# KaHIP/KaMinPar

Hardware: NVIDIA H100
Metric: lp_edges_per_second (higher is better)
Workload: dtype int32

## Files before the change

kaminpar_b200/csrc/lp_sweep.cuh:

```cuda
#pragma once

#include "lp_device.cuh"
#include "lp_sortnet.cuh"

namespace kmp {

template <int MODE>
__device__ __forceinline__ void emit_proposal(const SweepArgs &a, uint32_t idx, uint32_t u, uint32_t target,
                                              int32_t uw) {
  a.mv_u[idx] = u;
  a.mv_t[idx] = target;
  if (!a.accumulate) {
    return;
  }
  if (MODE == 0) {
    atomicAdd(&a.incoming[target], uw);
  } else {
    const uint32_t lvl = ladder_level(bijective32(u, a.base_commit));
    atomicAdd(&a.hist[target * kLadderLevels + lvl], uw);
  }
}

__device__ __forceinline__ void block_count_flush(const SweepArgs &a, unsigned long long edges,
                                                  unsigned long long nodes) {
  for (int o = 16; o > 0; o >>= 1) {
    edges += __shfl_xor_sync(kFull, edges, o);
    nodes += __shfl_xor_sync(kFull, nodes, o);
  }
  if ((threadIdx.x & 31) == 0 && nodes != 0) {
    atomicAdd(&a.counters[0], edges);
    atomicAdd(&a.counters[kCounterNodesOffset], nodes);
  }
}

template <bool P64>
__device__ __forceinline__ typename LabG<P64>::word load_labg(const SweepArgs &a, uint32_t v) {
  return static_cast<const typename LabG<P64>::word *>(a.labg)[v];
}

template <int R> struct ThreadRow {
  uint32_t u, beg, deg;
  uint32_t v[R > 0 ? R : 1];
};
template <int R> __device__ __forceinline__ void load_row(const SweepArgs &a, ThreadRow<R> &r) {
  r.beg = a.xadj[r.u];
  const uint32_t deg = a.xadj[r.u + 1] - r.beg;
  r.deg = deg > a.max_num_neighbors ? a.max_num_neighbors : deg;
#pragma unroll
  for (int j = 0; j < R; ++j) {
    r.v[j] = j < static_cast<int>(r.deg) ? a.adjncy[r.beg + j] : 0u;
  }
}

template <int MODE, bool EW, bool P64, int N, int R>
__device__ __forceinline__ bool sweep_thread_vertex(const SweepArgs &a, const ThreadRow<R> &r, bool flag,
                                                    unsigned long long &edges, unsigned long long &nodes,
                                                    uint32_t &target, int32_t &uw) {
  const uint32_t u = r.u;
  const uint32_t own = a.label[u];
  uw = a.vwgt != nullptr ? a.vwgt[u] : 1;
  const int32_t own_w = a.weight[own];
  uint32_t keys[N];
  int32_t ws[N];
  bool hit = false;
#pragma unroll
  for (int j = 0; j < N; ++j) {
    keys[j] = kEmpty;
    ws[j] = 0;
    if (j < static_cast<int>(r.deg)) {
      const uint32_t v = R > 0 ? r.v[j] : a.adjncy[r.beg + j];
      const typename LabG<P64>::word g = load_labg<P64>(a, v);
      hit = hit || stamp_hit(LabG<P64>::stamp(g), a.window);
      bool ok = true;
      if (MODE == 1 && a.communities != nullptr) {
        ok = a.communities[u] == a.communities[v];
      }
      if (ok) {
        keys[j] = LabG<P64>::label(g);
        ws[j] = EW ? a.adjwgt[r.beg + j] : 1;
      }
    }
  }
  if (!(flag || hit)) {
    return false;
  }
  edges += r.deg;
  nodes += 1;
  if (a.active != nullptr && flag) {
    a.active[u] = 0;
  }
  bool skip = false;
  if (MODE == 1) {
    const int32_t mn = a.min_w != nullptr ? a.min_w[own] : 0;
    skip = (own_w - uw) < mn;
  }
  const bool store_fav = (MODE == 0) && (uw == own_w) && (own_w <= a.max_cluster_weight / 2);
  Cand best = cand_none(), fav = cand_none();
  if (!skip) {
    sort_registers<N, EW>(keys, ws);
    bool lazy_done = false;
    if (MODE == 0) {
      Cand top = cand_none();
      int32_t run = 0;
#pragma unroll
      for (int j = 0; j < N; ++j) {
        run += EW ? ws[j] : 1;
        const bool last = (j == N - 1) || (keys[j + 1 < N ? j + 1 : j] != keys[j]);
        if (last) {
          const int32_t rating = run;
          run = 0;
          if (keys[j] != kEmpty && rating > 0) {
            if (rating >= top.gain) {
              const Cand x{rating, 0, tie_hash(a.base_tie, u, keys[j]), keys[j]};
              if (cand_better<0>(x, top)) {
                top = x;
              }
            }
            if (store_fav && rating >= fav.gain) {
              const Cand y{rating, 0, tie_hash(a.base_fav, u, keys[j]), keys[j]};
              if (cand_better<0>(y, fav)) {
                fav = y;
              }
            }
          }
        }
      }
      bool top_ok = true;
      if (top.gain > 0) {
        top_ok = (a.weight[top.key] + uw <= a.max_cluster_weight) || (top.key == own);
        if (a.communities != nullptr) {
          top_ok = top_ok && (a.communities[top.key] == a.communities[own]);
        }
      }
      if (top_ok) {
        best = top;
        lazy_done = true;
      }
    }
    if (!lazy_done) {
      int32_t run = 0;
#pragma unroll
      for (int j = 0; j < N; ++j) {
        run += EW ? ws[j] : 1;
        const bool last = (j == N - 1) || (keys[j + 1 < N ? j + 1 : j] != keys[j]);
        if (last) {
          const int32_t rating = run;
          run = 0;
          if (keys[j] != kEmpty) {
            Cand f;
            const Cand c = eval_candidate<MODE>(a, u, own, uw, own_w, keys[j], rating, MODE == 0 ? false : store_fav, f);
            if (cand_better<MODE>(c, best)) {
              best = c;
            }
          }
        }
      }
    }
  }
  return finish_vertex<MODE>(a, u, own, store_fav, best, fav, target);
}

template <int MODE>
__device__ __forceinline__ void emit_cta_iteration(const SweepArgs &a, bool proposes, uint32_t u, uint32_t target,
                                                   int32_t uw, uint32_t it, uint32_t (&s_cnt)[2][8],
                                                   uint32_t (&s_base)[2]) {
  const unsigned ballot = __ballot_sync(kFull, proposes);
  const int lane = threadIdx.x & 31;
  const int wib = threadIdx.x >> 5;
  const int par = it & 1;
  if (lane == 0) {
    s_cnt[par][wib] = static_cast<uint32_t>(__popc(ballot));
  }
  __syncthreads();
  if (threadIdx.x == 0) {
    uint32_t total = 0;
    for (int w = 0; w < 8; ++w) {
      total += s_cnt[par][w];
    }
    s_base[par] = total != 0 ? atomicAdd(a.mover_count, total) : 0u;
  }
  __syncthreads();
  if (proposes) {
    uint32_t idx = s_base[par] + __popc(ballot & ((1u << lane) - 1u));
    for (int w = 0; w < wib; ++w) {
      idx += s_cnt[par][w];
    }
    emit_proposal<MODE>(a, idx, u, target, uw);
  }
}

template <int MODE, bool EW, bool P64, int N> __global__ void __launch_bounds__(256) sweep_thread(const SweepArgs a) {
  __shared__ uint32_t s_cnt[2][8];
  __shared__ uint32_t s_base[2];
  unsigned long long edges = 0, nodes = 0;
  const uint32_t stride = gridDim.x * blockDim.x;
  const uint32_t bound = (a.list_size + 255u) & ~255u;
  uint32_t it = 0;
  for (uint32_t i = blockIdx.x * blockDim.x + threadIdx.x; i < bound; i += stride, ++it) {
    bool proposes = false;
    uint32_t target = 0;
    int32_t uw = 1;
    ThreadRow<0> r;
    r.u = 0;
    if (i < a.list_size) {
      r.u = a.list[i];
      const bool flag = a.active == nullptr || a.active[r.u] != 0;
      if (flag || a.pull) {
        load_row<0>(a, r);
        proposes = sweep_thread_vertex<MODE, EW, P64, N>(a, r, flag, edges, nodes, target, uw);
      }
    }
    emit_cta_iteration<MODE>(a, proposes, r.u, target, uw, it, s_cnt, s_base);
  }
  block_count_flush(a, edges, nodes);
}

__device__ __forceinline__ uint32_t pow2_ceil(uint32_t x) {
  return x <= 1 ? 1u : (1u << (32 - __clz(static_cast<int>(x - 1))));
}

__device__ __forceinline__ void table_add(uint32_t *keys, int32_t *vals, uint32_t mask, bool direct, uint32_t key,
                                          int32_t w) {
  uint32_t slot = direct ? key : (lowbias32(key) & mask);
  while (true) {
    const uint32_t prev = atomicCAS(&keys[slot], kEmpty, key);
    if (prev == kEmpty || prev == key) {
      atomicAdd(&vals[slot], w);
      return;
    }
    slot = (slot + 1) & mask;
  }
}

template <int T> struct TeamSync {
  static __device__ __forceinline__ void sync(int id) {
    if (T == 32) {
      __syncwarp();
    } else {
      asm volatile("bar.sync %0, %1;" ::"r"(id), "r"(T) : "memory");
    }
  }
  static __device__ __forceinline__ bool any(int id, bool p) {
    if (T == 32) {
      __syncwarp();
      return __any_sync(kFull, p);
    } else {
      int r;
      asm volatile(
          "{\n"
          ".reg .pred q, r;\n"
          "setp.ne.s32 q, %3, 0;\n"
          "bar.red.or.pred r, %1, %2, q;\n"
          "selp.s32 %0, 1, 0, r;\n"
          "}\n"
          : "=r"(r)
          : "r"(id), "r"(T), "r"(static_cast<int>(p))
          : "memory");
      return r != 0;
    }
  }
};

template <int MODE, int T>
__device__ __forceinline__ Cand team_argmax(int id, int tid, Cand c, Cand *s_red) {
  Cand r = warp_argmax<MODE>(kFull, c);
  if (T == 32) {
    return r;
  }
  TeamSync<T>::sync(id);
  if ((tid & 31) == 0) {
    s_red[tid >> 5] = r;
  }
  TeamSync<T>::sync(id);
  Cand x = cand_none();
  if ((tid & 31) < T / 32) {
    x = s_red[tid & 31];
  }
  return warp_argmax<MODE>(kFull, x);
}

template <bool V16> struct TeamVals;
template <> struct TeamVals<false> {
  using word = int32_t;
  static constexpr int kBytesPerSlot = 4;
  static __device__ __forceinline__ void add(word *v, uint32_t slot, int32_t w) { atomicAdd(&v[slot], w); }
  static __device__ __forceinline__ int32_t get(const word *v, uint32_t slot) { return v[slot]; }
  static __device__ __forceinline__ void clear(word *v, uint32_t slot) { v[slot] = 0; }
};
template <> struct TeamVals<true> {
  using word = uint32_t;
  static constexpr int kBytesPerSlot = 2;
  static __device__ __forceinline__ void add(word *v, uint32_t slot, int32_t w) {
    atomicAdd(&v[slot >> 1], static_cast<uint32_t>(w) << ((slot & 1u) * 16u));
  }
  static __device__ __forceinline__ int32_t get(const word *v, uint32_t slot) {
    return static_cast<int32_t>((v[slot >> 1] >> ((slot & 1u) * 16u)) & 0xFFFFu);
  }
  static __device__ __forceinline__ void clear(word *v, uint32_t slot) { reinterpret_cast<uint16_t *>(v)[slot] = 0; }
};

template <bool V16, bool EW>
__device__ __forceinline__ bool team_table_add(uint32_t *keys, typename TeamVals<V16>::word *vals, uint32_t mask,
                                               bool direct, uint32_t key, int32_t w, uint32_t &slot) {
  slot = direct ? key : (lowbias32(key) & mask);
  while (true) {
    const uint32_t prev = atomicCAS(&keys[slot], kEmpty, key);
    if (!EW && prev == kEmpty) {
      return true;
    }
    if (prev == kEmpty || prev == key) {
      TeamVals<V16>::add(vals, slot, w);
      return prev == kEmpty;
    }
    slot = (slot + 1) & mask;
  }
}
template <bool V16, bool EW>
__device__ __forceinline__ int32_t team_rating(const typename TeamVals<V16>::word *vals, uint32_t slot) {
  return TeamVals<V16>::get(vals, slot) + (EW ? 0 : 1);
}

template <int T> constexpr int team_ctas_per_sm() { return T == 32 ? 6 : T == 1024 ? 1 : 3; }

template <int MODE, bool EW, bool P64, int T, int SLOTS, int TEAMS, bool V16 = false>
__global__ void __launch_bounds__(T *TEAMS, team_ctas_per_sm<T>()) sweep_team(const SweepArgs a) {
  static_assert((SLOTS & (SLOTS - 1)) == 0, "table size must be a power of two");
  static_assert(SLOTS <= 65536, "claim lists hold 16-bit slot indices");
  static_assert(!(V16 && EW), "16-bit ratings need unit edge weights");
  using TV = TeamVals<V16>;
  constexpr int kListCap = SLOTS / 2;
  extern __shared__ __align__(16) unsigned char smem_raw[];
  __shared__ Cand s_red_all[TEAMS][T > 32 ? T / 32 : 1];
  __shared__ uint16_t s_list_all[TEAMS][kListCap];
  __shared__ uint32_t s_next[TEAMS], s_claims[TEAMS];
  __shared__ unsigned long long s_edges[TEAMS], s_nodes[TEAMS];
  const int team = threadIdx.x / T;
  const int tid = threadIdx.x % T;
  const int lane = threadIdx.x & 31;
  const int bar = 1 + team;
  uint32_t *keys = reinterpret_cast<uint32_t *>(smem_raw) + static_cast<size_t>(team) * SLOTS;
  typename TV::word *vals = reinterpret_cast<typename TV::word *>(
      smem_raw + sizeof(uint32_t) * SLOTS * TEAMS + static_cast<size_t>(team) * SLOTS * TV::kBytesPerSlot);
  Cand *s_red = s_red_all[team];
  uint16_t *list = s_list_all[team];
  for (int s = tid; s < SLOTS; s += T) {
    keys[s] = kEmpty;
    TV::clear(vals, s);
  }
  uint32_t next = 0;
  unsigned long long edges = 0, nodes = 0;
  if (tid == 0) {
    next = atomicAdd(a.queue, 1u);
    if (T > 32) {
      s_edges[team] = 0;
      s_nodes[team] = 0;
    }
  }
  TeamSync<T>::sync(bar);
  while (true) {
    uint32_t i;
    if (T == 32) {
      i = __shfl_sync(kFull, next, 0);
    } else {
      if (tid == 0) {
        s_next[team] = next;
        s_claims[team] = 0;
      }
      TeamSync<T>::sync(bar);
      i = s_next[team];
    }
    if (i >= a.list_size) {
      break;
    }
    if (tid == 0) {
      next = atomicAdd(a.queue, 1u);
    }
    const uint32_t u = a.list[i];
    const bool flag = a.active == nullptr || a.active[u] != 0;
    if (!flag && !a.pull) {
      TeamSync<T>::sync(bar);
      continue;
    }
    const uint32_t beg = a.xadj[u];
    uint32_t deg = a.xadj[u + 1] - beg;
    if (deg > a.max_num_neighbors) {
      deg = a.max_num_neighbors;
    }
    const uint32_t own = a.label[u];
    const int32_t uw = a.vwgt != nullptr ? a.vwgt[u] : 1;
    const int32_t own_w = a.weight[own];
    bool skip = false;
    if (MODE == 1) {
      const int32_t mn = a.min_w != nullptr ? a.min_w[own] : 0;
      skip = (own_w - uw) < mn;
    }
    const bool direct = a.num_labels <= static_cast<uint32_t>(SLOTS);
    bool hit = false;
    uint32_t claims = 0;
    constexpr int B = 4;
    for (uint32_t e0 = 0; e0 < deg; e0 += T * B) {
      uint32_t kb[B];
      int32_t wb[B];
      uint32_t vb[B];
#pragma unroll
      for (int j = 0; j < B; ++j) {
        const uint32_t e = e0 + j * T + tid;
        vb[j] = e < deg ? a.adjncy[beg + e] : kEmpty;
        wb[j] = (EW && e < deg) ? a.adjwgt[beg + e] : 1;
      }
#pragma unroll
      for (int j = 0; j < B; ++j) {
        kb[j] = kEmpty;
        if (vb[j] != kEmpty) {
          const typename LabG<P64>::word g = load_labg<P64>(a, vb[j]);
          hit = hit || stamp_hit(LabG<P64>::stamp(g), a.window);
          bool ok = !skip;
          if (MODE == 1 && a.communities != nullptr) {
            ok = ok && a.communities[u] == a.communities[vb[j]];
          }
          if (ok) {
            kb[j] = LabG<P64>::label(g);
          }
        }
      }
      uint32_t sl[B];
      unsigned claimed[B];
#pragma unroll
      for (int j = 0; j < B; ++j) {
        sl[j] = 0;
        claimed[j] = __ballot_sync(kFull, kb[j] != kEmpty && team_table_add<V16, EW>(keys, vals, SLOTS - 1, direct,
                                                                                     kb[j], wb[j], sl[j]));
      }
      uint32_t n = 0;
#pragma unroll
      for (int j = 0; j < B; ++j) {
        n += __popc(claimed[j]);
      }
      if (n != 0) {
        uint32_t base = claims;
        if (T == 32) {
          claims += n;
        } else {
          if (lane == 0) {
            base = atomicAdd(&s_claims[team], n);
          }
          base = __shfl_sync(kFull, base, 0);
        }
        const unsigned below = (1u << lane) - 1u;
#pragma unroll
        for (int j = 0; j < B; ++j) {
          if ((claimed[j] >> lane) & 1u) {
            list[base + __popc(claimed[j] & below)] = static_cast<uint16_t>(sl[j]);
          }
          base += __popc(claimed[j]);
        }
      }
    }
    const bool any_hit = TeamSync<T>::any(bar, hit);
    const bool act = flag || any_hit;
    const uint32_t nc = T == 32 ? claims : s_claims[team];
    const bool store_fav = (MODE == 0) && (uw == own_w) && (own_w <= a.max_cluster_weight / 2);
    Cand best = cand_none(), fav = cand_none();
    if (act) {
      Cand c = cand_none(), f = cand_none();
      if (MODE == 0) {
        for (uint32_t l = tid; l < nc; l += T) {
          const uint32_t s = list[l];
          const uint32_t k = keys[s];
          const int32_t r = team_rating<V16, EW>(vals, s);
          if (r >= c.gain) {
            Cand x{r, 0, tie_hash(a.base_tie, u, k), k};
            if (cand_better<0>(x, c)) {
              c = x;
            }
          }
          if (store_fav && r >= f.gain) {
            Cand y{r, 0, tie_hash(a.base_fav, u, k), k};
            if (cand_better<0>(y, f)) {
              f = y;
            }
          }
        }
        const Cand top = team_argmax<0, T>(bar, tid, c, s_red);
        if (store_fav) {
          fav = team_argmax<0, T>(bar, tid, f, s_red);
        }
        bool top_ok = true;
        if (top.gain > 0) {
          top_ok = (a.weight[top.key] + uw <= a.max_cluster_weight) || (top.key == own);
          if (a.communities != nullptr) {
            top_ok = top_ok && (a.communities[top.key] == a.communities[own]);
          }
        }
        if (top_ok) {
          best = top;
        } else {
          Cand cb = cand_none();
          for (uint32_t l0 = 0; l0 < nc; l0 += T * 4) {
            uint32_t kk[4];
            int32_t rr[4], ww[4];
#pragma unroll
            for (int j = 0; j < 4; ++j) {
              const uint32_t l = l0 + j * T + tid;
              const uint32_t s = l < nc ? list[l] : 0u;
              kk[j] = l < nc ? keys[s] : kEmpty;
              rr[j] = l < nc ? team_rating<V16, EW>(vals, s) : 0;
            }
#pragma unroll
            for (int j = 0; j < 4; ++j) {
              ww[j] = kk[j] != kEmpty ? a.weight[kk[j]] : 0;
            }
#pragma unroll
            for (int j = 0; j < 4; ++j) {
              if (kk[j] != kEmpty) {
                Cand ff;
                const Cand cc = eval_candidate_w<0>(a, u, own, uw, own_w, kk[j], rr[j], ww[j], false, ff);
                if (cand_better<0>(cc, cb)) {
                  cb = cc;
                }
              }
            }
          }
          best = team_argmax<0, T>(bar, tid, cb, s_red);
        }
      } else {
        for (uint32_t l = tid; l < nc; l += T) {
          const uint32_t s = list[l];
          const uint32_t k = keys[s];
          Cand ff;
          const Cand cc = eval_candidate_w<1>(a, u, own, uw, own_w, k, team_rating<V16, EW>(vals, s), a.weight[k], false, ff);
          if (cand_better<1>(cc, c)) {
            c = cc;
          }
        }
        best = team_argmax<1, T>(bar, tid, c, s_red);
      }
    }
    for (uint32_t l = tid; l < nc; l += T) {
      const uint32_t s = list[l];
      keys[s] = kEmpty;
      TV::clear(vals, s);
    }
    if (act && tid == 0) {
      if (T == 32) {
        edges += deg;
        nodes += 1;
      } else {
        s_edges[team] += deg;
        s_nodes[team] += 1;
      }
      if (a.active != nullptr && flag) {
        a.active[u] = 0;
      }
      uint32_t target;
      if (finish_vertex<MODE>(a, u, own, store_fav, best, fav, target)) {
        const uint32_t idx = atomicAdd(a.mover_count, 1u);
        emit_proposal<MODE>(a, idx, u, target, uw);
      }
    }
    TeamSync<T>::sync(bar);
  }
  if (T > 32 && tid == 0) {
    edges = s_edges[team];
    nodes = s_nodes[team];
  }
  if (tid == 0 && nodes != 0) {
    atomicAdd(&a.counters[0], edges);
    atomicAdd(&a.counters[kCounterNodesOffset], nodes);
  }
}

constexpr int kChunkEdges = 2048;
constexpr int kSliceEdges = 256;
constexpr int kSliceTableSlots = 512;
constexpr int kChunkThreads = 256;
constexpr uint32_t kBucketCap = 512;
constexpr uint32_t kBucketTargetFill = 256;
constexpr uint32_t kSelTableSlots = 1024;
constexpr int kSelWarps = 4;

struct HubOverflow {
  uint32_t bucket;
  uint32_t key;
  int32_t rating;
  uint32_t pad;
};

struct HubArgs {
  const uint32_t *__restrict__ item_entry;
  const uint32_t *__restrict__ item_chunk;
  const uint32_t *__restrict__ item_u;
  const uint32_t *__restrict__ item_beg;
  const uint32_t *__restrict__ item_deg;
  uint32_t num_items;
  const uint32_t *__restrict__ table_off;
  unsigned long long *__restrict__ g_tab;
  uint32_t *__restrict__ cursor;
  HubOverflow *__restrict__ ovf;
  uint32_t *__restrict__ ovf_count;
  uint32_t ovf_cap;
  uint32_t bucket_cap;
  uint32_t sel_limit;
  uint32_t stage_adjncy;
  const uint32_t *__restrict__ sel_entry;
  const uint32_t *__restrict__ sel_piece;
  uint32_t num_sel_items;
  const uint32_t *__restrict__ sel_begin;
  Cand *__restrict__ part_best;
  Cand *__restrict__ part_fav;
  uint32_t rank, world;
  uint32_t *__restrict__ queue;
  uint32_t *__restrict__ hit;
  uint32_t *__restrict__ lab;
  const uint32_t *__restrict__ lab_off;
  const uint32_t *__restrict__ item_cls;
};

__host__ __device__ __forceinline__ uint32_t hub_buckets(uint32_t full_degree) {
  const uint32_t need = (full_degree + kBucketTargetFill - 1) / kBucketTargetFill;
  uint32_t p = 1;
  while (p < need) {
    p <<= 1;
  }
  return p;
}

__device__ __forceinline__ uint32_t smem_u32(const void *p) {
  return static_cast<uint32_t>(__cvta_generic_to_shared(p));
}
__device__ __forceinline__ void mbar_init(uint64_t *bar, uint32_t count) {
  asm volatile("mbarrier.init.shared::cta.b64 [%0], %1;" ::"r"(smem_u32(bar)), "r"(count) : "memory");
}
__device__ __forceinline__ void mbar_arrive_expect_tx(uint64_t *bar, uint32_t bytes) {
  asm volatile("mbarrier.arrive.expect_tx.shared::cta.b64 _, [%0], %1;" ::"r"(smem_u32(bar)), "r"(bytes) : "memory");
}
__device__ __forceinline__ void mbar_wait(uint64_t *bar, uint32_t parity) {
  asm volatile(
      "{\n"
      ".reg .pred p;\n"
      "WAIT_LOOP:\n"
      "mbarrier.try_wait.parity.shared::cta.b64 p, [%0], %1;\n"
      "@p bra DONE;\n"
      "bra WAIT_LOOP;\n"
      "DONE:\n"
      "}\n" ::"r"(smem_u32(bar)),
      "r"(parity)
      : "memory");
}
__device__ __forceinline__ void tma_load_1d(void *dst_smem, const void *src_gmem, uint32_t bytes, uint64_t *bar) {
  asm volatile("cp.async.bulk.shared::cluster.global.mbarrier::complete_tx::bytes [%0], [%1], %2, [%3];" ::"r"(
                   smem_u32(dst_smem)),
               "l"(src_gmem), "r"(bytes), "r"(smem_u32(bar))
               : "memory");
}

struct HubItem {
  uint32_t valid;
  uint32_t u;
  uint32_t entry;
  uint32_t full_deg;
  uint32_t gbeg, gend;
  uint32_t a0;
  uint32_t staged;
};

__device__ __forceinline__ void mbar_arrive(uint64_t *bar) {
  asm volatile("mbarrier.arrive.shared::cta.b64 _, [%0];" ::"r"(smem_u32(bar)) : "memory");
}

constexpr int kHubStages = 2;
constexpr int kHubConsumerWarps = kChunkThreads / 32;
constexpr int kHubThreads = kChunkThreads + 32;
constexpr int kHubScatterSmem = kHubConsumerWarps * kSliceTableSlots * 8;

template <int MODE, bool EW, bool P64>
__global__ void __launch_bounds__(kHubThreads, 4) sweep_hub_scatter(const SweepArgs a, const HubArgs hb, uint32_t m_total) {
  extern __shared__ __align__(16) unsigned char smem_raw[];
  constexpr int kAllSlots = kHubConsumerWarps * kSliceTableSlots;
  uint32_t *all_keys = reinterpret_cast<uint32_t *>(smem_raw);
  int32_t *all_vals = reinterpret_cast<int32_t *>(smem_raw + sizeof(uint32_t) * kAllSlots);
  __shared__ __align__(16) uint32_t s_adj[kHubStages][kChunkEdges + 8];
  __shared__ __align__(8) uint64_t s_full[kHubStages];
  __shared__ __align__(8) uint64_t s_empty[kHubStages];
  __shared__ HubItem s_item[kHubStages];
  const int lane = threadIdx.x & 31;
  const int wib = threadIdx.x >> 5;
  if (threadIdx.x == 0) {
    for (int s = 0; s < kHubStages; ++s) {
      mbar_init(&s_full[s], 1);
      mbar_init(&s_empty[s], kHubConsumerWarps);
    }
    asm volatile("fence.mbarrier_init.release.cluster;" ::: "memory");
  }
  for (int s = threadIdx.x; s < kAllSlots; s += kHubThreads) {
    all_keys[s] = kEmpty;
    all_vals[s] = 0;
  }
  __syncthreads();

  if (wib == kHubConsumerWarps) {
    if (lane == 0) {
      for (uint32_t k = 0;; ++k) {
        const int stage = static_cast<int>(k % kHubStages);
        const uint32_t round = k / kHubStages;
        mbar_wait(&s_empty[stage], (round & 1u) ^ 1u);
        const uint32_t it = atomicAdd(hb.queue, 1u);
        HubItem d{};
        d.valid = 0;
        if (it >= hb.num_items) {
          d.valid = 2;
          s_item[stage] = d;
          mbar_arrive(&s_full[stage]);
          break;
        }
        const uint32_t entry = hb.item_entry[it];
        const uint32_t u = hb.item_u[it];
        const uint32_t beg0 = hb.item_beg[it];
        const uint32_t full_deg = hb.item_deg[it];
        const uint32_t chunk = hb.item_chunk[it];
        if (entry % hb.world == hb.rank && (a.active == nullptr || a.pull || a.active[u] != 0)) {
          uint32_t deg = full_deg;
          if (deg > a.max_num_neighbors) {
            deg = a.max_num_neighbors;
          }
          const uint32_t cbeg = chunk * kChunkEdges;
          bool ok = cbeg < deg;
          if (ok && MODE == 1) {
            const uint32_t own = a.label[u];
            const int32_t uw = a.vwgt != nullptr ? a.vwgt[u] : 1;
            const int32_t mn = a.min_w != nullptr ? a.min_w[own] : 0;
            ok = !((a.weight[own] - uw) < mn);
          }
          if (ok) {
            const uint32_t cend = (cbeg + kChunkEdges < deg) ? cbeg + kChunkEdges : deg;
            d.valid = 1;
            d.u = u;
            d.entry = entry;
            d.full_deg = full_deg;
            d.gbeg = beg0 + cbeg;
            d.gend = beg0 + cend;
            d.a0 = d.gbeg & ~3u;
            d.staged = 0;
            if (hb.stage_adjncy) {
              uint32_t a1 = (d.gend + 3u) & ~3u;
              const uint32_t m4 = m_total & ~3u;
              if (a1 > m4) {
                a1 = m4;
              }
              d.staged = a1 > d.a0 ? a1 - d.a0 : 0;
            }
          }
        }
        s_item[stage] = d;
        if (d.valid && d.staged > 0) {
          asm volatile("fence.proxy.async.shared::cta;" ::: "memory");
          mbar_arrive_expect_tx(&s_full[stage], d.staged * 4);
          tma_load_1d(&s_adj[stage][0], a.adjncy + d.a0, d.staged * 4, &s_full[stage]);
        } else {
          mbar_arrive(&s_full[stage]);
        }
      }
    }
    return;
  }

  uint32_t *keys = all_keys + wib * kSliceTableSlots;
  int32_t *vals = all_vals + wib * kSliceTableSlots;
  for (uint32_t k = 0;; ++k) {
    const int stage = static_cast<int>(k % kHubStages);
    const uint32_t round = k / kHubStages;
    mbar_wait(&s_full[stage], round & 1u);
    const HubItem d = s_item[stage];
    if (d.valid == 2) {
      break;
    }
    const uint32_t wbeg = d.gbeg + wib * kSliceEdges;
    const bool mine = d.valid && wbeg < d.gend;
    if (mine) {
      const uint32_t wend = wbeg + kSliceEdges < d.gend ? wbeg + kSliceEdges : d.gend;
      const uint32_t staged_end = d.a0 + d.staged;
      bool hit = false;
      for (uint32_t e0 = wbeg; e0 < wend; e0 += 128) {
        uint32_t k4[4];
        int32_t w4[4];
#pragma unroll
        for (int j = 0; j < 4; ++j) {
          const uint32_t e = e0 + j * 32 + lane;
          k4[j] = kEmpty;
          w4[j] = 0;
          if (e < wend) {
            const uint32_t v = e < staged_end ? s_adj[stage][e - d.a0] : a.adjncy[e];
            bool ok = true;
            if (MODE == 1 && a.communities != nullptr) {
              ok = a.communities[d.u] == a.communities[v];
            }
            const typename LabG<P64>::word g = load_labg<P64>(a, v);
            hit = hit || stamp_hit(LabG<P64>::stamp(g), a.window);
            if (ok) {
              k4[j] = LabG<P64>::label(g);
              w4[j] = EW ? a.adjwgt[e] : 1;
            }
          }
        }
#pragma unroll
        for (int j = 0; j < 4; ++j) {
          if (k4[j] != kEmpty) {
            table_add(keys, vals, kSliceTableSlots - 1, false, k4[j], w4[j]);
          }
        }
      }
      if (a.pull && __any_sync(kFull, hit) && lane == 0) {
        atomicOr(&hb.hit[d.entry], 1u);
      }
    }
    __syncwarp();
    if (lane == 0) {
      mbar_arrive(&s_empty[stage]);
    }
    if (mine) {
      const uint32_t pmask = hub_buckets(d.full_deg) - 1;
      const uint32_t bucket0 = hb.table_off[d.entry];
      constexpr int B = 4;
      for (uint32_t s0 = lane; s0 < kSliceTableSlots; s0 += 32 * B) {
        uint32_t kk[B], bb[B], pos[B];
        int32_t rr[B];
#pragma unroll
        for (int j = 0; j < B; ++j) {
          const uint32_t s = s0 + j * 32;
          kk[j] = keys[s];
          rr[j] = vals[s];
          if (kk[j] != kEmpty) {
            keys[s] = kEmpty;
            vals[s] = 0;
          }
        }
#pragma unroll
        for (int j = 0; j < B; ++j) {
          bb[j] = bucket0 + (lowbias32(kk[j]) & pmask);
          pos[j] = kk[j] != kEmpty ? atomicAdd(&hb.cursor[bb[j]], 1u) : 0u;
        }
#pragma unroll
        for (int j = 0; j < B; ++j) {
          if (kk[j] != kEmpty) {
            if (pos[j] < hb.bucket_cap) {
              hb.g_tab[static_cast<size_t>(bb[j]) * kBucketCap + pos[j]] =
                  (static_cast<unsigned long long>(kk[j]) << 32) | static_cast<uint32_t>(rr[j]);
            } else {
              const uint32_t o = atomicAdd(hb.ovf_count, 1u);
              if (o < hb.ovf_cap) {
                hb.ovf[o] = HubOverflow{bb[j], kk[j], rr[j], 0u};
              }
            }
          }
        }
      }
      __syncwarp();
    }
  }
}

template <int MODE> __global__ void __launch_bounds__(kSelWarps * 32) sweep_hub_select(const SweepArgs a, const HubArgs hb) {
  static_assert(MODE == 1, "the clusterer rates its hubs with sweep_hub_rate");
  __shared__ uint32_t s_keys[kSelWarps][kSelTableSlots];
  __shared__ int32_t s_vals[kSelWarps][kSelTableSlots];
  __shared__ uint32_t s_claims_all[kSelWarps];
  const int lane = threadIdx.x & 31;
  const int wib = threadIdx.x >> 5;
  uint32_t *keys = s_keys[wib];
  int32_t *vals = s_vals[wib];
  uint32_t *s_claims = &s_claims_all[wib];
  for (uint32_t s = lane; s < kSelTableSlots; s += 32) {
    keys[s] = kEmpty;
    vals[s] = 0;
  }
  if (lane == 0) {
    *s_claims = 0;
  }
  __syncwarp();
  const uint32_t nwarps = gridDim.x * kSelWarps;
  for (uint32_t it = blockIdx.x * kSelWarps + wib; it < hb.num_sel_items; it += nwarps) {
    const uint32_t entry = hb.sel_entry[it];
    const uint32_t u = a.list[entry];
    Cand c = cand_none();
    const bool act = (entry % hb.world == hb.rank) && (a.active == nullptr || a.pull || a.active[u] != 0);
    const uint32_t b = hb.table_off[entry] + hb.sel_piece[it];
    const uint32_t appended = act ? __ldcg(&hb.cursor[b]) : 0u;
    if (appended != 0) {
      const uint32_t full_deg = a.xadj[u + 1] - a.xadj[u];
      const uint32_t pbits = 31 - __clz(static_cast<int>(hub_buckets(full_deg)));
      const uint32_t own = a.label[u];
      const int32_t uw = a.vwgt != nullptr ? a.vwgt[u] : 1;
      const int32_t own_w = a.weight[own];
      const uint32_t n_reg = appended < hb.bucket_cap ? appended : hb.bucket_cap;
      const uint32_t n_ovf = appended > hb.bucket_cap ? min(__ldcg(hb.ovf_count), hb.ovf_cap) : 0u;
      uint32_t tcap = pow2_ceil(2 * appended);
      tcap = tcap < 64 ? 64u : tcap > kSelTableSlots ? kSelTableSlots : tcap;
      const uint32_t tmask = tcap - 1;
      const uint32_t full_limit = tcap / 2 + tcap / 8;
      const uint32_t limit = (hb.sel_limit != 0 && hb.sel_limit < full_limit) ? hb.sel_limit : full_limit;
      const unsigned long long *reg = hb.g_tab + static_cast<size_t>(b) * kBucketCap;
      auto insert = [&](uint32_t key, int32_t r) {
        uint32_t slot = lowbias32(key ^ 0x9E3779B9u) & tmask;
        while (true) {
          const uint32_t prev = atomicCAS(&keys[slot], kEmpty, key);
          if (prev == kEmpty) {
            atomicAdd(s_claims, 1u);
          }
          if (prev == kEmpty || prev == key) {
            atomicAdd(&vals[slot], r);
            return;
          }
          slot = (slot + 1) & tmask;
        }
      };
      uint32_t K = 1;
      while (true) {
        c = cand_none();
        bool overflowed = false;
        for (uint32_t cls = 0; cls < K && !overflowed; ++cls) {
          constexpr int B = 4;
          for (uint32_t i0 = 0; i0 < n_reg && !overflowed; i0 += 32 * B) {
            unsigned long long e[B];
#pragma unroll
            for (int j = 0; j < B; ++j) {
              const uint32_t i = i0 + j * 32 + lane;
              e[j] = i < n_reg ? __ldcs(reg + i) : ~0ull;
            }
#pragma unroll
            for (int j = 0; j < B; ++j) {
              const uint32_t key = static_cast<uint32_t>(e[j] >> 32);
              if (key != kEmpty && ((lowbias32(key) >> pbits) & (K - 1)) == cls) {
                insert(key, static_cast<int32_t>(static_cast<uint32_t>(e[j])));
              }
            }
            if (n_ovf != 0) {
              __syncwarp();
              overflowed = *s_claims > limit;
              __syncwarp();
            }
          }
          for (uint32_t i0 = 0; i0 < n_ovf && !overflowed; i0 += 32 * B) {
#pragma unroll
            for (int j = 0; j < B; ++j) {
              const uint32_t i = i0 + j * 32 + lane;
              if (i < n_ovf) {
                const HubOverflow o = hb.ovf[i];
                if (o.bucket == b && ((lowbias32(o.key) >> pbits) & (K - 1)) == cls) {
                  insert(o.key, o.rating);
                }
              }
            }
            __syncwarp();
            overflowed = *s_claims > limit;
            __syncwarp();
          }
          __syncwarp();
          const bool evaluate = !overflowed;
          for (uint32_t s0 = 0; s0 < tcap; s0 += 32 * B) {
            uint32_t kk[B];
            int32_t rr[B], ww[B];
#pragma unroll
            for (int j = 0; j < B; ++j) {
              const uint32_t s = s0 + j * 32 + lane;
              kk[j] = s < tcap ? keys[s] : kEmpty;
              rr[j] = kk[j] != kEmpty ? vals[s] : 0;
            }
#pragma unroll
            for (int j = 0; j < B; ++j) {
              ww[j] = (kk[j] != kEmpty && evaluate) ? a.weight[kk[j]] : 0;
            }
#pragma unroll
            for (int j = 0; j < B; ++j) {
              if (kk[j] != kEmpty) {
                const uint32_t s = s0 + j * 32 + lane;
                keys[s] = kEmpty;
                vals[s] = 0;
                if (evaluate) {
                  Cand ff;
                  const Cand cc = eval_candidate_w<1>(a, u, own, uw, own_w, kk[j], rr[j], ww[j], false, ff);
                  if (cand_better<1>(cc, c)) {
                    c = cc;
                  }
                }
              }
            }
          }
          __syncwarp();
          if (lane == 0) {
            *s_claims = 0;
          }
          __syncwarp();
        }
        if (!overflowed) {
          break;
        }
        K <<= 1;
      }
      if (lane == 0) {
        hb.cursor[b] = 0;
      }
    }
    const Cand best = warp_argmax<1>(kFull, c);
    if (lane == 0) {
      hb.part_best[it] = best;
    }
  }
}

constexpr int kRateThreads = 1024;
constexpr uint32_t kRateSlots = 16384;
constexpr uint32_t kRateListCap = kRateSlots / 2;
constexpr uint32_t kHubClassEdges = 8192;
constexpr uint32_t kRateStage = 64;
template <bool EW> constexpr int rate_smem() {
  return static_cast<int>(kRateSlots * 8 + kRateListCap * 2 + (kRateThreads / 32) * kRateStage * (EW ? 8 : 4));
}

__host__ __device__ __forceinline__ uint32_t hub_classes(uint32_t full_degree) {
  const uint32_t need = (full_degree + kHubClassEdges - 1) / kHubClassEdges;
  uint32_t p = 1;
  while (p < need) {
    p <<= 1;
  }
  return p;
}

template <bool P64> __global__ void __launch_bounds__(256) sweep_hub_gather(const SweepArgs a, const HubArgs hb) {
  constexpr int B = kChunkEdges / 256;
  const int lane = threadIdx.x & 31;
  for (uint32_t it = blockIdx.x; it < hb.num_items; it += gridDim.x) {
    const uint32_t entry = hb.item_entry[it];
    const uint32_t u = hb.item_u[it];
    if (entry % hb.world != hb.rank || !(a.active == nullptr || a.pull || a.active[u] != 0)) {
      continue;
    }
    const uint32_t deg = min(hb.item_deg[it], a.max_num_neighbors);
    const uint32_t cbeg = hb.item_chunk[it] * kChunkEdges;
    if (cbeg >= deg) {
      continue;
    }
    const uint32_t cend = min(cbeg + kChunkEdges, deg);
    const uint32_t *adj = a.adjncy + hb.item_beg[it];
    uint32_t *out = hb.lab + hb.lab_off[entry];
    uint32_t v[B];
#pragma unroll
    for (int j = 0; j < B; ++j) {
      const uint32_t e = cbeg + j * 256 + threadIdx.x;
      v[j] = e < cend ? adj[e] : kEmpty;
    }
    bool hit = false;
#pragma unroll
    for (int j = 0; j < B; ++j) {
      if (v[j] != kEmpty) {
        const typename LabG<P64>::word g = load_labg<P64>(a, v[j]);
        hit = hit || stamp_hit(LabG<P64>::stamp(g), a.window);
        out[cbeg + j * 256 + threadIdx.x] = LabG<P64>::label(g);
      }
    }
    if (a.pull && __any_sync(kFull, hit) && lane == 0) {
      atomicOr(&hb.hit[entry], 1u);
    }
  }
}

template <bool EW>
__device__ __forceinline__ bool rate_insert(uint32_t *keys, int32_t *vals, uint16_t *list, uint32_t *s_claims,
                                            uint32_t limit, uint32_t key, int32_t w, bool valid, int lane) {
  uint32_t slot = 0;
  bool claimed = false;
  if (valid) {
    slot = lowbias32(key ^ 0x9E3779B9u) & (kRateSlots - 1);
    while (true) {
      const uint32_t prev = atomicCAS(&keys[slot], kEmpty, key);
      if (prev == kEmpty || prev == key) {
        claimed = prev == kEmpty;
        if (EW || !claimed) {
          atomicAdd(&vals[slot], w);
        }
        break;
      }
      slot = (slot + 1) & (kRateSlots - 1);
    }
  }
  const unsigned mask = __ballot_sync(kFull, claimed);
  if (mask == 0) {
    return false;
  }
  const uint32_t n = __popc(mask);
  uint32_t base = 0;
  if (lane == 0) {
    base = atomicAdd(s_claims, n);
  }
  base = __shfl_sync(kFull, base, 0);
  const uint32_t idx = base + __popc(mask & ((1u << lane) - 1u));
  if (claimed && idx < kRateListCap) {
    list[idx] = static_cast<uint16_t>(slot);
  }
  return base + n > limit;
}

template <bool EW> __global__ void __launch_bounds__(kRateThreads, 1) sweep_hub_rate(const SweepArgs a, const HubArgs hb) {
  constexpr int T = kRateThreads;
  constexpr int kWarps = T / 32;
  constexpr int B = 8;
  extern __shared__ __align__(16) unsigned char smem_raw[];
  uint32_t *keys = reinterpret_cast<uint32_t *>(smem_raw);
  int32_t *vals = reinterpret_cast<int32_t *>(smem_raw + sizeof(uint32_t) * kRateSlots);
  uint32_t *stage_k = reinterpret_cast<uint32_t *>(smem_raw + 8 * kRateSlots);
  int32_t *stage_w = reinterpret_cast<int32_t *>(stage_k + kWarps * kRateStage);
  uint16_t *list = reinterpret_cast<uint16_t *>(stage_k + (EW ? 2 : 1) * kWarps * kRateStage);
  __shared__ Cand s_red[kWarps];
  __shared__ uint32_t s_item, s_claims;
  const int tid = threadIdx.x;
  const int lane = tid & 31;
  const int wib = tid >> 5;
  const unsigned below = (1u << lane) - 1u;
  uint32_t *stk = stage_k + wib * kRateStage;
  int32_t *stw = stage_w + wib * kRateStage;
  for (uint32_t s = tid; s < kRateSlots; s += T) {
    keys[s] = kEmpty;
    vals[s] = 0;
  }
  const uint32_t limit = (hb.sel_limit != 0 && hb.sel_limit < kRateListCap) ? max(hb.sel_limit, 2u) : kRateListCap;
  while (true) {
    if (tid == 0) {
      s_item = atomicAdd(hb.queue, 1u);
    }
    __syncthreads();
    const uint32_t it = s_item;
    if (it >= hb.num_items) {
      break;
    }
    const uint32_t entry = hb.item_entry[it];
    const uint32_t c0 = hb.item_cls[it];
    const uint32_t u = a.list[entry];
    if (entry % hb.world == hb.rank && (a.active == nullptr || a.pull || a.active[u] != 0)) {
      const uint32_t beg = a.xadj[u];
      const uint32_t full_deg = a.xadj[u + 1] - beg;
      const uint32_t deg = min(full_deg, a.max_num_neighbors);
      const uint32_t K0 = hub_classes(full_deg);
      const uint32_t own = a.label[u];
      const int32_t uw = a.vwgt != nullptr ? a.vwgt[u] : 1;
      const int32_t own_w = a.weight[own];
      const bool store_fav = (uw == own_w) && (own_w <= a.max_cluster_weight / 2);
      const uint32_t *lab = hb.lab + hb.lab_off[entry];
      Cand best = cand_none(), fav = cand_none();
      uint32_t cls = c0, K = K0;
      while (true) {
        if (tid == 0) {
          s_claims = 0;
        }
        __syncthreads();
        bool wover = false;
        uint32_t head = 0, pend = 0;
        for (uint32_t e0 = wib * 32 * B; e0 < deg && !wover; e0 += T * B) {
          uint32_t kb[B];
#pragma unroll
          for (int j = 0; j < B; ++j) {
            const uint32_t e = e0 + j * 32 + lane;
            kb[j] = e < deg ? __ldcg(lab + e) : kEmpty;
          }
#pragma unroll
          for (int j = 0; j < B; ++j) {
            if (!wover) {
              const bool in = kb[j] != kEmpty && (lowbias32(kb[j]) & (K - 1)) == cls;
              const unsigned m = __ballot_sync(kFull, in);
              if (in) {
                const uint32_t pos = (head + pend + __popc(m & below)) & (kRateStage - 1);
                stk[pos] = kb[j];
                if (EW) {
                  stw[pos] = a.adjwgt[beg + e0 + j * 32 + lane];
                }
              }
              pend += __popc(m);
              if (pend >= 32) {
                __syncwarp();
                const uint32_t sl = (head + lane) & (kRateStage - 1);
                wover = rate_insert<EW>(keys, vals, list, &s_claims, limit, stk[sl], EW ? stw[sl] : 1, true, lane);
                __syncwarp();
                head = (head + 32) & (kRateStage - 1);
                pend -= 32;
              }
            }
          }
        }
        if (!wover) {
          __syncwarp();
          const bool v = lane < pend;
          const uint32_t sl = (head + lane) & (kRateStage - 1);
          wover = rate_insert<EW>(keys, vals, list, &s_claims, limit, v ? stk[sl] : 0u, (EW && v) ? stw[sl] : 1, v, lane);
        }
        const bool over = __syncthreads_or(wover);
        if (over) {
          for (uint32_t s = tid; s < kRateSlots; s += T) {
            keys[s] = kEmpty;
            vals[s] = 0;
          }
          K <<= 1;
          __syncthreads();
          continue;
        }
        const uint32_t nc = s_claims;
        Cand c = cand_none(), f = cand_none();
        for (uint32_t l = tid; l < nc; l += T) {
          const uint32_t s = list[l];
          const uint32_t k = keys[s];
          const int32_t r = vals[s] + (EW ? 0 : 1);
          if (r > 0 && r >= c.gain) {
            const Cand x{r, 0, tie_hash(a.base_tie, u, k), k};
            if (cand_better<0>(x, c)) {
              c = x;
            }
          }
          if (store_fav && r > 0 && r >= f.gain) {
            const Cand y{r, 0, tie_hash(a.base_fav, u, k), k};
            if (cand_better<0>(y, f)) {
              f = y;
            }
          }
        }
        Cand cb = team_argmax<0, T>(1, tid, c, s_red);
        if (store_fav) {
          const Cand cf = team_argmax<0, T>(1, tid, f, s_red);
          if (cand_better<0>(cf, fav)) {
            fav = cf;
          }
        }
        bool top_ok = true;
        if (cb.gain > 0) {
          top_ok = (a.weight[cb.key] + uw <= a.max_cluster_weight) || (cb.key == own);
          if (a.communities != nullptr) {
            top_ok = top_ok && (a.communities[cb.key] == a.communities[own]);
          }
        }
        if (!top_ok) {
          Cand ce = cand_none();
          for (uint32_t l0 = 0; l0 < nc; l0 += T * 4) {
            uint32_t kk[4];
            int32_t rr[4], ww[4];
#pragma unroll
            for (int j = 0; j < 4; ++j) {
              const uint32_t l = l0 + j * T + tid;
              const uint32_t s = l < nc ? list[l] : 0u;
              kk[j] = l < nc ? keys[s] : kEmpty;
              rr[j] = l < nc ? vals[s] + (EW ? 0 : 1) : 0;
            }
#pragma unroll
            for (int j = 0; j < 4; ++j) {
              ww[j] = kk[j] != kEmpty ? a.weight[kk[j]] : 0;
            }
#pragma unroll
            for (int j = 0; j < 4; ++j) {
              if (kk[j] != kEmpty) {
                Cand ff;
                const Cand cc = eval_candidate_w<0>(a, u, own, uw, own_w, kk[j], rr[j], ww[j], false, ff);
                if (cand_better<0>(cc, ce)) {
                  ce = cc;
                }
              }
            }
          }
          cb = team_argmax<0, T>(1, tid, ce, s_red);
        }
        if (cand_better<0>(cb, best)) {
          best = cb;
        }
        for (uint32_t l = tid; l < nc; l += T) {
          const uint32_t s = list[l];
          keys[s] = kEmpty;
          vals[s] = 0;
        }
        __syncthreads();
        bool done = true;
        while (K > K0) {
          const uint32_t half = K >> 1;
          if ((cls & half) == 0) {
            cls |= half;
            done = false;
            break;
          }
          cls &= ~half;
          K = half;
        }
        if (done) {
          break;
        }
      }
      if (tid == 0) {
        hb.part_best[hb.sel_begin[entry] + c0] = best;
        hb.part_fav[hb.sel_begin[entry] + c0] = fav;
      }
    }
    __syncthreads();
  }
}

template <int MODE> __global__ void __launch_bounds__(256) sweep_hub_final(const SweepArgs a, const HubArgs hb) {
  const int lane = threadIdx.x & 31;
  const uint32_t warp = (blockIdx.x * blockDim.x + threadIdx.x) >> 5;
  const uint32_t nwarps = (gridDim.x * blockDim.x) >> 5;
  unsigned long long edges = 0, nodes = 0;
  for (uint32_t i = warp; i < a.list_size; i += nwarps) {
    if (i % hb.world != hb.rank) {
      continue;
    }
    const uint32_t u = a.list[i];
    bool flag = true;
    if (a.active != nullptr) {
      int fl = 0, ht = 0;
      if (lane == 0) {
        fl = static_cast<int>(a.active[u]);
        if (a.pull) {
          ht = static_cast<int>(hb.hit[i]);
          hb.hit[i] = 0;
        }
      }
      fl = __shfl_sync(kFull, fl, 0);
      ht = __shfl_sync(kFull, ht, 0);
      flag = fl != 0;
      if (fl == 0 && ht == 0) {
        continue;
      }
    }
    const uint32_t full_deg = a.xadj[u + 1] - a.xadj[u];
    uint32_t deg = full_deg;
    if (deg > a.max_num_neighbors) {
      deg = a.max_num_neighbors;
    }
    const uint32_t own = a.label[u];
    const int32_t uw = a.vwgt != nullptr ? a.vwgt[u] : 1;
    const int32_t own_w = a.weight[own];
    const uint32_t pieces = MODE == 0 ? hub_classes(full_deg) : hub_buckets(full_deg);
    const uint32_t first = hb.sel_begin[i];
    const bool store_fav = (MODE == 0) && (uw == own_w) && (own_w <= a.max_cluster_weight / 2);
    Cand c = cand_none(), f = cand_none();
    for (uint32_t q = lane; q < pieces; q += 32) {
      const Cand pb = hb.part_best[first + q];
      if (cand_better<MODE>(pb, c)) {
        c = pb;
      }
      if (MODE == 0) {
        const Cand pf = hb.part_fav[first + q];
        if (cand_better<0>(pf, f)) {
          f = pf;
        }
      }
    }
    const Cand best = warp_argmax<MODE>(kFull, c);
    const Cand fav = (MODE == 0) ? warp_argmax<0>(kFull, f) : cand_none();
    if (lane == 0) {
      edges += deg;
      nodes += 1;
      if (a.active != nullptr && flag) {
        a.active[u] = 0;
      }
      uint32_t target;
      if (finish_vertex<MODE>(a, u, own, store_fav, best, fav, target)) {
        const uint32_t idx = atomicAdd(a.mover_count, 1u);
        emit_proposal<MODE>(a, idx, u, target, uw);
      }
    }
  }
  block_count_flush(a, edges, nodes);
}

}
```

Baseline: 43.50 billion.

## Prefetch next vertex metadata across warp lanes and claim two queue items

```diff
diff --git a/kaminpar_b200/csrc/lp_sweep.cuh b/kaminpar_b200/csrc/lp_sweep.cuh
--- a/kaminpar_b200/csrc/lp_sweep.cuh
+++ b/kaminpar_b200/csrc/lp_sweep.cuh
@@ -349,44 +349,91 @@
   }
   uint32_t next = 0;
   unsigned long long edges = 0, nodes = 0;
+  constexpr uint32_t kPending = 0xFFFFFFFEu;
+  auto row_vertex = [&]() {
+    const uint32_t j = __shfl_sync(kFull, next, 0);
+    if (lane == 5) {
+      next = next == kPending ? j + 1 : next;
+    } else {
+      next = j < a.list_size ? a.list[j] : kEmpty;
+    }
+  };
+  auto row_fields = [&]() {
+    const uint32_t v = next;
+    if (v != kEmpty) {
+      if (lane < 2) {
+        next = a.xadj[v + lane];
+      } else if (lane == 3) {
+        next = a.active == nullptr ? 1u : a.active[v];
+      } else if (lane == 4) {
+        next = a.label[v];
+      }
+    }
+  };
   if (tid == 0) {
-    next = atomicAdd(a.queue, 1u);
+    next = atomicAdd(a.queue, T == 32 ? 2u : 1u);
     if (T > 32) {
       s_edges[team] = 0;
       s_nodes[team] = 0;
     }
   }
+  if constexpr (T == 32) {
+    if (lane == 5) {
+      next = kPending;
+    }
+    row_vertex();
+    row_fields();
+  }
   TeamSync<T>::sync(bar);
   while (true) {
-    uint32_t i;
-    if (T == 32) {
-      i = __shfl_sync(kFull, next, 0);
+    uint32_t u, beg, deg, own;
+    bool flag;
+    if constexpr (T == 32) {
+      u = __shfl_sync(kFull, next, 2);
+      if (u == kEmpty) {
+        break;
+      }
+      beg = __shfl_sync(kFull, next, 0);
+      deg = __shfl_sync(kFull, next, 1) - beg;
+      flag = __shfl_sync(kFull, next, 3) != 0;
+      own = __shfl_sync(kFull, next, 4);
+      const uint32_t spare = __shfl_sync(kFull, next, 5);
+      if (lane == 0) {
+        next = spare != kEmpty ? spare : atomicAdd(a.queue, 2u);
+      } else if (lane == 5) {
+        next = spare != kEmpty ? kEmpty : kPending;
+      }
+      if (!flag && !a.pull) {
+        row_vertex();
+        row_fields();
+        continue;
+      }
     } else {
       if (tid == 0) {
         s_next[team] = next;
         s_claims[team] = 0;
       }
       TeamSync<T>::sync(bar);
-      i = s_next[team];
-    }
-    if (i >= a.list_size) {
-      break;
-    }
-    if (tid == 0) {
-      next = atomicAdd(a.queue, 1u);
-    }
-    const uint32_t u = a.list[i];
-    const bool flag = a.active == nullptr || a.active[u] != 0;
-    if (!flag && !a.pull) {
-      TeamSync<T>::sync(bar);
-      continue;
-    }
-    const uint32_t beg = a.xadj[u];
-    uint32_t deg = a.xadj[u + 1] - beg;
+      const uint32_t i = s_next[team];
+      if (i >= a.list_size) {
+        break;
+      }
+      if (tid == 0) {
+        next = atomicAdd(a.queue, 1u);
+      }
+      u = a.list[i];
+      flag = a.active == nullptr || a.active[u] != 0;
+      if (!flag && !a.pull) {
+        TeamSync<T>::sync(bar);
+        continue;
+      }
+      beg = a.xadj[u];
+      deg = a.xadj[u + 1] - beg;
+      own = a.label[u];
+    }
     if (deg > a.max_num_neighbors) {
       deg = a.max_num_neighbors;
     }
-    const uint32_t own = a.label[u];
     const int32_t uw = a.vwgt != nullptr ? a.vwgt[u] : 1;
     const int32_t own_w = a.weight[own];
     bool skip = false;
@@ -455,6 +502,9 @@
           base += __popc(claimed[j]);
         }
       }
+    }
+    if constexpr (T == 32) {
+      row_vertex();
     }
     const bool any_hit = TeamSync<T>::any(bar, hit);
     const bool act = flag || any_hit;
@@ -535,6 +585,9 @@
         }
         best = team_argmax<1, T>(bar, tid, c, s_red);
       }
+    }
+    if constexpr (T == 32) {
+      row_fields();
     }
     for (uint32_t l = tid; l < nc; l += T) {
       const uint32_t s = list[l];
```

New measurement: 44.73 billion (median of 6 runs). +2.8%, better.
